# Keytoyze/Mug-Diffusion

Measured on NVIDIA H100. Metric: denoising-steps/sec, higher is better.
Workload: dtype f32

## Files before the change

### mug_diffusion_b200/csrc/gemm_tc.cu

```cuda
#include "gemm_tc.cuh"

namespace mugd {

template <int BN, int EPI>
__global__ void __launch_bounds__(TC_THREADS, 1)
gemm_tc_kernel(const __grid_constant__ CUtensorMap tmA, const __grid_constant__ CUtensorMap tmA1,
               const __grid_constant__ CUtensorMap tmA2, const __grid_constant__ CUtensorMap tmB, const __grid_constant__ CUtensorMap tmWhi,
               const __grid_constant__ CUtensorMap tmWlo, const __grid_constant__ TcParams p) {
    extern __shared__ uint8_t smem_raw[];
    const uint32_t base = (smem_u32(smem_raw) + 1023u) & ~1023u;
    const TcBars<BN> B(base);
    TC_STAMP(p, 0, blockIdx.x == 0 && blockIdx.y == 0 && blockIdx.z == 0);
    if (threadIdx.x < 32) {
        B.init_parallel((int)threadIdx.x);
    } else if (threadIdx.x < 38) {
        const CUtensorMap* m = threadIdx.x == 32 ? &tmA : threadIdx.x == 33 ? &tmA1 : threadIdx.x == 34 ? &tmA2
                             : threadIdx.x == 35 ? &tmB : threadIdx.x == 36 ? &tmWhi : &tmWlo;
        asm volatile("prefetch.tensormap [%0];" ::"l"(reinterpret_cast<uint64_t>(m)) : "memory");
    }
    __syncthreads();
    TC_STAMP(p, 1, blockIdx.x == 0 && blockIdx.y == 0 && blockIdx.z == 0);
    gemm_tc_tile<BN, EPI>(&tmA, &tmA1, &tmA2, &tmB, &tmWhi, &tmWlo, p, blockIdx.x, blockIdx.y, blockIdx.z, base);
}

template <int BN, int EPI>
__global__ void __launch_bounds__(TC_THREADS)
gemm_tc_reduce_kernel(const __grid_constant__ TcParams p) {
    tc_reduce<BN, EPI>(p, blockIdx.x);
}

#ifdef MUGD_TC_TIMELINE
static long long* g_tc_dbg = nullptr;
#endif
static float g_tc_kstep128 = 0.55f;
static float g_tc_split = 3.0f;
static int g_tc_force_bn = 0;

static bool tc_shape_ok(const mugd_gemm& g) {
    if (!(g.conv_mode == MUGD_CONV_NONE || g.conv_mode == MUGD_CONV_SAME || g.conv_mode == MUGD_CONV_DOWN ||
          g.conv_mode == MUGD_CONV_TAPS)) return false;
    if (g.conv_mode == MUGD_CONV_DOWN && g.Lout < 2) return false;
    if (g.K2 % TC_BK != 0 || (g.K2 > 0 && g.conv_mode == MUGD_CONV_DOWN)) return false;
    return g.K % TC_BK == 0 && g.N >= 16 && g.N % 4 == 0;
}

bool gemm_tc_supported(const mugd_gemm& g) {
    if (!tc_shape_ok(g)) return false;
    if (!g.W_hi || !g.W_lo) return false;
    if (g.lda % 4 != 0 || !aligned16(g.A) || !aligned16(g.W_hi) || !aligned16(g.W_lo)) return false;
    if (g.K2 > 0 && (!g.A2 || g.lda2 % 4 != 0 || !aligned16(g.A2))) return false;
    return true;
}

static int tc_validate_fusions(const mugd_gemm& g) {
    if (g.row_moments)
        MUGD_REQUIRE(g.act == MUGD_ACT_NONE && g.gate == MUGD_GATE_NONE && !g.ln_stats && (reinterpret_cast<uintptr_t>(g.row_moments) & 15u) == 0,
                     "gemm: row_moments needs act == gate == NONE, no folded LayerNorm and a 16-byte aligned buffer");
    if (g.ln_stats) {
        MUGD_REQUIRE(g.ln_colsum && aligned16(g.ln_colsum) && (reinterpret_cast<uintptr_t>(g.ln_stats) & 15u) == 0 && g.taps == 1 && g.K2 == 0 &&
                         g.act == MUGD_ACT_NONE && (g.gate == MUGD_GATE_NONE || g.gate == MUGD_GATE_GEGLU) && !g.rowvec,
                     "gemm: folded LayerNorm needs a single-source Linear with act NONE and gate NONE/GEGLU");
    }
    return MUGD_OK;
}

TcGeometry tc_geometry(const mugd_gemm& g, int sm_count, int forced_split) {
    TcGeometry t = {};
    TcParams::Hot& h = t.hot;
    t.BN = (g.N >= 128) ? 128 : 64;
    if (g.conv_mode == MUGD_CONV_NONE) { h.Lrows = g.M; h.Bs = 1; }
    else { h.Lrows = g.Lout; h.Bs = g.M / g.Lout; }
    if (h.Lrows >= TC_BM) {
        h.box_l = TC_BM; h.box_b = 1;
        h.tiles_per_sample = (h.Lrows + TC_BM - 1) / TC_BM;
        t.gy = h.tiles_per_sample * h.Bs;
    } else {
        h.box_l = h.Lrows;
        h.box_b = TC_BM / h.Lrows;
        if (h.box_b > h.Bs) h.box_b = h.Bs;
        h.tiles_per_sample = 1;
        t.gy = (h.Bs + h.box_b - 1) / h.box_b;
    }
    h.kblocks = g.K / TC_BK;
    h.it_main = g.taps * h.kblocks;
    h.total_it = h.it_main + g.K2 / TC_BK;
    int splits = 1;
    float best = 1e30f;
    static const int cands[2] = {64, 128};
    for (int cand = 0; cand < 2; ++cand) {
        const int bn = cands[cand];
        if (bn > 64 && g.N < bn) continue;
        if (bn == 64 && g.N >= 128 && g_tc_force_bn != 64) continue;
        if (g_tc_force_bn && bn != g_tc_force_bn && !(g_tc_force_bn > g.N && bn == 64)) continue;
        const int gx = (g.N + bn - 1) / bn;
        const int tiles = gx * t.gy;
        const float kstep = bn == 128 ? g_tc_kstep128 : 0.4f;
        const int sp_max = forced_split > 0 ? forced_split : (tiles < sm_count ? 16 : 1);
        for (int sp = forced_split > 0 ? forced_split : 1; sp <= sp_max && sp <= h.total_it; ++sp) {
            const int per = (h.total_it + sp - 1) / sp;
            if (forced_split <= 0 && sp > 1 && per < 2) break;
            if (forced_split <= 0 && sp > 1 && tiles * sp > 2 * sm_count) break;
            const int waves = (tiles * sp + sm_count - 1) / sm_count;
            const float est = waves * (1.0f + kstep * per) + (sp > 1 ? g_tc_split : 0.0f);
            if (est < best - 0.25f) { best = est; splits = sp; t.BN = bn; }
        }
    }
    h.gx = (g.N + t.BN - 1) / t.BN;
    if (splits > h.total_it) splits = h.total_it;
    if (splits < 1) splits = 1;
    h.splits = splits;
    h.it_base = h.total_it / splits;
    h.it_rem = h.total_it % splits;
    h.conv_mode = g.conv_mode;
    h.tap_shift = g.tap_shift;
    h.tap_dilation = g.tap_dilation;
    t.ws_floats = splits > 1 ? (int64_t)h.gx * t.gy * splits * TC_BM * t.BN : 0;
    return t;
}

int tc_plan(const DeviceInfo& dev, const mugd_gemm& g, const mugd_gemm* next, TcPlanned* out) {
    MUGD_REQUIRE(gemm_tc_supported(g), "gemm_tc: unsupported shape/operands");
    int rc = tc_validate_fusions(g);
    if (rc != MUGD_OK) return rc;
    const TcGeometry t = tc_geometry(g, dev.sm_count, g.split_k);
    const TcParams::Hot& h = t.hot;
    if (h.splits > 1) {
        MUGD_REQUIRE(g.workspace, "gemm_tc: split-K needs a workspace");
        MUGD_REQUIRE(g.workspace_bytes >= t.ws_floats * 4, "gemm_tc: workspace too small (%lld < %lld)", (long long)g.workspace_bytes,
                     (long long)t.ws_floats * 4);
    }
    const cuuint32_t a_box[3] = {(cuuint32_t)TC_BK, (cuuint32_t)h.box_l, (cuuint32_t)h.box_b};
    for (int tap = 0; tap < 3; ++tap) {
        if (tap > 0 && g.conv_mode != MUGD_CONV_DOWN) { out->maps[tap] = out->maps[0]; continue; }
        const bool down = g.conv_mode == MUGD_CONV_DOWN;
        const cuuint64_t rows = down ? (cuuint64_t)(h.Lrows - (tap == 2 ? 1 : 0)) : (cuuint64_t)h.Lrows;
        const cuuint64_t sample_rows = down ? (cuuint64_t)g.Lin : (cuuint64_t)h.Lrows;
        const cuuint64_t dims[3] = {(cuuint64_t)g.K, rows, (cuuint64_t)h.Bs};
        const cuuint64_t strides[2] = {(cuuint64_t)g.lda * 4 * (down ? 2 : 1), sample_rows * (cuuint64_t)g.lda * 4};
        rc = encode_f32_tma(&out->maps[tap], g.A + (down ? (int64_t)tap * g.lda : 0), 3, dims, strides, a_box, CU_TENSOR_MAP_L2_PROMOTION_L2_128B,
                            "gemm_tc A");
        if (rc != MUGD_OK) return rc;
    }
    if (g.K2 > 0) {
        const cuuint64_t dims[3] = {(cuuint64_t)g.K2, (cuuint64_t)h.Lrows, (cuuint64_t)h.Bs};
        const cuuint64_t strides[2] = {(cuuint64_t)g.lda2 * 4, (cuuint64_t)h.Lrows * (cuuint64_t)g.lda2 * 4};
        rc = encode_f32_tma(&out->maps[3], g.A2, 3, dims, strides, a_box, CU_TENSOR_MAP_L2_PROMOTION_L2_128B, "gemm_tc A2");
        if (rc != MUGD_OK) return rc;
    } else {
        out->maps[3] = out->maps[0];
    }
    const cuuint64_t ktot = (cuuint64_t)g.taps * g.K + g.K2;
    const cuuint64_t w_dims[2] = {ktot, (cuuint64_t)g.N};
    const cuuint64_t w_strides[1] = {ktot * 4};
    const cuuint32_t w_box[2] = {(cuuint32_t)TC_BK, (cuuint32_t)t.BN};
    for (int w = 0; w < 2; ++w) {
        rc = encode_f32_tma(&out->maps[4 + w], w == 0 ? g.W_hi : g.W_lo, 2, w_dims, w_strides, w_box, CU_TENSOR_MAP_L2_PROMOTION_L2_256B,
                            "gemm_tc W");
        if (rc != MUGD_OK) return rc;
    }
    TcParams& p = out->p;
    memset(&p, 0, sizeof(p));
    p.hot = h;
    p.hot.single_pass = dev.tc_single_pass ? 1 : 0;
    p.g = g;
    p.ws = (float*)g.workspace;
    p.gy = t.gy;
    p.ln_invK = 1.0 / (double)g.K;
    if (next) {
        p.pf_hi = next->W_hi;
        p.pf_lo = p.hot.single_pass ? nullptr : next->W_lo;
        p.pf_bytes = (int64_t)next->N * ((int64_t)next->taps * next->K + next->K2) * 4;
    }
#ifdef MUGD_TC_TIMELINE
    p.dbg = g_tc_dbg;
#endif
    out->BN = t.BN;
    return MUGD_OK;
}

template <int BN, int EPI>
static int tc_launch(const TcPlanned& pl, cudaStream_t st) {
    const TcParams& p = pl.p;
    const TcParams::Hot& h = p.hot;
    if (h.splits > 1) {
        MUGD_CHECK_CUDA(launch_k(gemm_tc_kernel<BN, TC_E_NONE>, dim3(h.gx, p.gy, h.splits), dim3(TC_THREADS), TcSmem<BN>::TOTAL, st, pl.maps[0],
                                 pl.maps[1], pl.maps[2], pl.maps[3], pl.maps[4], pl.maps[5], p));
        MUGD_CHECK_CUDA(launch_k(gemm_tc_reduce_kernel<BN, EPI>, dim3((unsigned)(h.gx * p.gy * (TC_BM / TC_RED_ROWS<BN>))), dim3(TC_THREADS), 0,
                                 st, p));
        return MUGD_OK;
    }
    MUGD_CHECK_CUDA(launch_k(gemm_tc_kernel<BN, EPI>, dim3(h.gx, p.gy, 1), dim3(TC_THREADS), TcSmem<BN>::TOTAL, st, pl.maps[0], pl.maps[1],
                             pl.maps[2], pl.maps[3], pl.maps[4], pl.maps[5], p));
    return MUGD_OK;
}

template <int BN, int... EPI>
static cudaError_t allow_smem_bn(int bytes, std::integer_sequence<int, EPI...>) {
    return allow_dynamic_smem(bytes, gemm_tc_kernel<BN, EPI>...);
}
cudaError_t gemm_tc_allow_smem(int bytes) {
    const cudaError_t e = allow_smem_bn<64>(bytes, std::make_integer_sequence<int, TC_E_COUNT>{});
    return e != cudaSuccess ? e : allow_smem_bn<128>(bytes, std::make_integer_sequence<int, TC_E_COUNT>{});
}

template <int BN>
static int tc_launch_bn(const TcPlanned& pl, cudaStream_t st) {
    switch (tc_epi_of(pl.p.g)) {
        case TC_E_GEGLU: return tc_launch<BN, TC_E_GEGLU>(pl, st);
        case TC_E_GLU: return tc_launch<BN, TC_E_GLU>(pl, st);
        case TC_E_SILU: return tc_launch<BN, TC_E_SILU>(pl, st);
        case TC_E_GELU: return tc_launch<BN, TC_E_GELU>(pl, st);
        case TC_E_SINK: return tc_launch<BN, TC_E_SINK>(pl, st);
        case TC_E_LN: return tc_launch<BN, TC_E_LN>(pl, st);
        case TC_E_LN_GEGLU: return tc_launch<BN, TC_E_LN_GEGLU>(pl, st);
        default: return tc_launch<BN, TC_E_NONE>(pl, st);
    }
}

int launch_gemm_tc(const DeviceInfo& dev, const mugd_gemm& g, const mugd_gemm* next, cudaStream_t st, int* launches) {
    TcPlanned pl;
    int rc = tc_plan(dev, g, next, &pl);
    if (rc != MUGD_OK) return rc;
    if (pl.BN == 128) rc = tc_launch_bn<128>(pl, st);
    else rc = tc_launch_bn<64>(pl, st);
    if (rc != MUGD_OK) return rc;
    if (launches) *launches += pl.p.hot.splits > 1 ? 2 : 1;
    return MUGD_OK;
}

}

extern "C" int mugd_debug_set_tc_cost(float kstep128_us, float kstep256_us, float split_us, float two_cta_fixed_us) {
    (void)kstep256_us;
    (void)two_cta_fixed_us;
    if (kstep128_us > 0.f) mugd::g_tc_kstep128 = kstep128_us;
    if (split_us > 0.f) mugd::g_tc_split = split_us;
    return MUGD_OK;
}

extern "C" int mugd_debug_set_tc_tile_n(int bn) {
    mugd::g_tc_force_bn = (bn == 64 || bn == 128) ? bn : 0;
    return MUGD_OK;
}

extern "C" int mugd_debug_set_tc_timing(long long* device_buf) {
#ifdef MUGD_TC_TIMELINE
    mugd::g_tc_dbg = device_buf;
    return MUGD_OK;
#else
    (void)device_buf;
    mugd::set_error("mugd_debug_set_tc_timing: this build has no timeline hooks (rebuild with -DMUGD_TC_TIMELINE, tools/build_variant.py)");
    return MUGD_ERR_INVALID;
#endif
}

extern "C" int mugd_gemm_tc_variant(const mugd_gemm* g, int32_t sm_count, int32_t* tile_n, int32_t* ctas_per_sm, int32_t* grid_ctas) {
    using namespace mugd;
    MUGD_REQUIRE(g, "gemm_tc_variant: null");
    if (!tc_shape_ok(*g)) {
        if (tile_n) *tile_n = 0;
        if (ctas_per_sm) *ctas_per_sm = 0;
        if (grid_ctas) *grid_ctas = 0;
        return MUGD_OK;
    }
    const int sms = sm_count > 0 ? sm_count : 132;
    const TcGeometry t = tc_geometry(*g, sms, g->split_k);
    if (tile_n) *tile_n = t.BN;
    if (ctas_per_sm) *ctas_per_sm = 1;
    if (grid_ctas) *grid_ctas = t.hot.gx * t.gy * t.hot.splits;
    return MUGD_OK;
}

extern "C" int mugd_gemm_tc_query(mugd_handle*, const mugd_gemm* g, int32_t sm_count, int32_t* supported, int32_t* splits,
                                  int64_t* workspace_bytes, int32_t* n_tiles) {
    using namespace mugd;
    MUGD_REQUIRE(g, "gemm_tc_query: null");
    const bool ok = tc_shape_ok(*g);
    if (supported) *supported = ok ? 1 : 0;
    if (!ok) {
        if (splits) *splits = 0;
        if (workspace_bytes) *workspace_bytes = 0;
        if (n_tiles) *n_tiles = 0;
        return MUGD_OK;
    }
    const TcGeometry t = tc_geometry(*g, sm_count > 0 ? sm_count : 132, g->split_k);
    if (splits) *splits = t.hot.splits;
    if (workspace_bytes) *workspace_bytes = t.ws_floats * 4;
    if (n_tiles) *n_tiles = t.hot.gx * t.gy;
    return MUGD_OK;
}
```

### mug_diffusion_b200/csrc/gemm_tc.cuh

```cuda
#pragma once
#include <cuda.h>
#include <stddef.h>

#include <type_traits>

#include "common.cuh"
#include "wgmma.cuh"

namespace mugd {

constexpr int TC_BM = 128;
constexpr int TC_BK = 32;
constexpr int TC_THREADS = 256;
constexpr uint32_t TC_A_BYTES = TC_BM * TC_BK * 4;

struct TcParams {
    struct Hot {
        int32_t Lrows, Bs;
        int32_t box_l, box_b;
        int32_t tiles_per_sample;
        int32_t it_base, it_rem;
        int32_t it_main;
        int32_t kblocks;
        int32_t total_it;
        int32_t splits;
        int32_t single_pass;
        int32_t conv_mode, tap_shift, tap_dilation;
        int32_t gx;
    } hot;
    mugd_gemm g;
    float* ws;
    int32_t gy;
    double ln_invK;
    const float* pf_hi;
    const float* pf_lo;
    int64_t pf_bytes;
#ifdef MUGD_TC_TIMELINE
    long long* dbg;
#endif
};
static_assert(sizeof(TcParams::Hot) == 64 && offsetof(TcParams, hot) == 0, "the hot fields are the first 64 bytes of the parameters");

#ifdef __CUDACC__
__device__ __forceinline__ long long gtimer() {
    long long t;
    asm volatile("mov.u64 %0, %%globaltimer;" : "=l"(t) :: "memory");
    return t;
}
#ifdef MUGD_TC_TIMELINE
#define TC_STAMP(p, k, cta0) do { if ((p).dbg && (cta0) && threadIdx.x == 0) (p).dbg[k] = gtimer(); } while (0)
#else
#define TC_STAMP(p, k, cta0) do { } while (0)
#endif
template <int BN>
struct TcSmem {
    static_assert(BN == 64 || BN == 128, "tile widths of the wgmma kernel");
    static constexpr uint32_t B_BYTES = BN * TC_BK * 4;
    static constexpr uint32_t STAGE_BYTES = TC_A_BYTES + 2 * B_BYTES;
    static constexpr int STAGES = BN == 128 ? 4 : 6;
    static constexpr uint32_t TILE_BYTES = STAGES * STAGE_BYTES;
    static constexpr uint32_t BAR_BYTES = 256;
    static constexpr uint32_t TOTAL = TILE_BYTES + 1024  + BAR_BYTES;
    static_assert(TOTAL <= 227u * 1024u, "shared memory budget");
    static_assert(128u * (BN + 4) * 4u + 1024u <= TILE_BYTES, "the staged accumulator tile + row statistics must fit the pipeline buffers");
};

template <int SEG>
__device__ __forceinline__ void tc_row_sink(double* buf, int m, float4 v) {
    float s = (v.x + v.y) + (v.z + v.w);
    float ss = (v.x * v.x + v.y * v.y) + (v.z * v.z + v.w * v.w);
#pragma unroll
    for (int o = SEG / 2; o > 0; o >>= 1) {
        s += __shfl_xor_sync(0xffffffffu, s, o);
        ss += __shfl_xor_sync(0xffffffffu, ss, o);
    }
    if ((threadIdx.x & (SEG - 1)) == 0 && m >= 0) {
        atomicAdd(buf + (int64_t)m * 2, (double)s);
        atomicAdd(buf + (int64_t)m * 2 + 1, (double)ss);
    }
}
__device__ __forceinline__ float2 tc_ln_from_moments(double s, double ss, double invK, float eps) {
    const double mean = s * invK;
    double var = ss * invK - mean * mean;
    const float v = fmaxf((float)var, 0.f) + eps;
    float r = rsqrtf(v);
    r = r * (1.5f - 0.5f * v * r * r);
    return make_float2((float)mean, r);
}

constexpr int TC_EPI_PLAIN = 0, TC_EPI_SINK = 1 , TC_EPI_LN = 2 ;

template <int ACT, int GATE, bool LNF>
__device__ __forceinline__ float4 tc_finish4(const mugd_gemm& g, float* dst, float4 acc, float4 bia, float4 rvv, float4 res, float4 cs, float2 ln,
                                             int m, int no) {
    float x[4];
    if constexpr (LNF) {
        x[0] = (acc.x - ln.x * cs.x) * ln.y + bia.x + rvv.x; x[1] = (acc.y - ln.x * cs.y) * ln.y + bia.y + rvv.y;
        x[2] = (acc.z - ln.x * cs.z) * ln.y + bia.z + rvv.z; x[3] = (acc.w - ln.x * cs.w) * ln.y + bia.w + rvv.w;
    } else {
        x[0] = acc.x + bia.x + rvv.x; x[1] = acc.y + bia.y + rvv.y; x[2] = acc.z + bia.z + rvv.z; x[3] = acc.w + bia.w + rvv.w;
    }
    if constexpr (ACT == MUGD_ACT_SILU) {
#pragma unroll
        for (int j = 0; j < 4; ++j) x[j] = silu_f(x[j]);
    } else if constexpr (ACT == MUGD_ACT_GELU) {
#pragma unroll
        for (int j = 0; j < 4; ++j) x[j] = gelu_f(x[j]);
    }
    if constexpr (GATE == MUGD_GATE_NONE) {
        const float4 o = make_float4(x[0] + res.x, x[1] + res.y, x[2] + res.z, x[3] + res.w);
        st_f4(dst, o);
        return o;
    } else {
        float o0, o1;
        if constexpr (GATE == MUGD_GATE_GEGLU) { o0 = x[0] * gelu_f(x[1]); o1 = x[2] * gelu_f(x[3]); }
        else { o0 = x[0] * sigmoid_f(x[1]); o1 = x[2] * sigmoid_f(x[3]); }
        if (g.residual) {
            const float2 rr = *reinterpret_cast<const float2*>(g.residual + (int64_t)m * g.ldr + no);
            o0 += rr.x; o1 += rr.y;
        }
        *reinterpret_cast<float2*>(dst) = make_float2(o0, o1);
        return make_float4(o0, o1, 0.f, 0.f);
    }
}

template <int BN, int ACT, int GATE, int MODE>
__device__ __forceinline__ void tc_store_tile(const mugd_gemm& g, uint32_t stage, int m_base, int n0, int rows_valid, const float* rowvec,
                                              uint32_t rowstat, float4 bia, float4 cs) {
    constexpr int SP = BN + 4;
    constexpr int C4 = BN / 4;
    constexpr int NU = TC_BM * C4 / TC_THREADS;
    constexpr int U = NU < 16 ? NU : 16;
    constexpr int SEG = C4 < 32 ? C4 : 32;
    static_assert(TC_THREADS % C4 == 0, "a thread keeps its column quad for the whole tile");
    const int c4 = (int)threadIdx.x % C4;
    const int nn = n0 + c4 * 4;
    const bool col_ok = nn < g.N;
    const bool has_res = GATE == MUGD_GATE_NONE && g.residual != nullptr;
    constexpr int RPP = TC_THREADS / C4;
    const int row0 = (int)threadIdx.x / C4;
    const int n_rows = min(rows_valid, g.M - m_base);
    const int no = (GATE == MUGD_GATE_NONE) ? nn : (nn >> 1);
    float* cp = g.C + (int64_t)(m_base + row0) * g.ldc + no;
    const float* rp = has_res ? g.residual + (int64_t)(m_base + row0) * g.ldr + nn : nullptr;
    const int64_t c_step = (int64_t)RPP * g.ldc, r_step = (int64_t)RPP * g.ldr;
    int smp = 0, smp_end = 0;
    if (rowvec) { smp = (m_base + row0) / g.Lout; smp_end = (smp + 1) * g.Lout; }
    auto pass = [&](auto full_tag) {
        constexpr bool FULL = decltype(full_tag)::value;
#pragma unroll 1
        for (int i0 = 0; i0 < NU; i0 += U) {
            float4 res[U], rvv[U];
#pragma unroll
            for (int u = 0; u < U; ++u) {
                const int row = row0 + (i0 + u) * RPP;
                res[u] = rvv[u] = make_float4(0.f, 0.f, 0.f, 0.f);
                if (FULL || (row < n_rows && col_ok)) {
                    if (has_res) res[u] = ld_f4(rp + (int64_t)(i0 + u) * r_step);
                    if (rowvec) {
                        const int m = m_base + row;
                        while (m >= smp_end) { ++smp; smp_end += g.Lout; }
                        rvv[u] = ld_f4(rowvec + (int64_t)smp * g.rowvec_b_stride + nn);
                    }
                }
            }
#pragma unroll
            for (int u = 0; u < U; ++u) {
                const int row = row0 + (i0 + u) * RPP;
                const int m = m_base + row;
                const bool ok = FULL || (row < n_rows && col_ok);
                const float4 acc = lds_f4(stage + (uint32_t)(row * SP + c4 * 4) * 4u);
                float2 ln = make_float2(0.f, 1.f);
                if constexpr (MODE == TC_EPI_LN) ln = lds_f2(rowstat + (uint32_t)row * 8u);
                float4 o = make_float4(0.f, 0.f, 0.f, 0.f);
                if (ok) o = tc_finish4<ACT, GATE, MODE == TC_EPI_LN>(g, cp + (int64_t)(i0 + u) * c_step, acc, bia, rvv[u], res[u], cs, ln, m, no);
                if constexpr (MODE == TC_EPI_SINK) tc_row_sink<SEG>(g.row_moments, ok ? m : -1, o);
            }
        }
    };
    if (n_rows >= TC_BM && n0 + BN <= g.N) pass(std::true_type{});
    else pass(std::false_type{});
}

enum TcEpi { TC_E_NONE = 0, TC_E_GEGLU, TC_E_GLU, TC_E_SILU, TC_E_GELU, TC_E_SINK, TC_E_LN, TC_E_LN_GEGLU, TC_E_COUNT };
template <int EPI> struct TcEpiTraits;
template <> struct TcEpiTraits<TC_E_NONE>     { static constexpr int ACT = MUGD_ACT_NONE, GATE = MUGD_GATE_NONE,  MODE = TC_EPI_PLAIN; };
template <> struct TcEpiTraits<TC_E_GEGLU>    { static constexpr int ACT = MUGD_ACT_NONE, GATE = MUGD_GATE_GEGLU, MODE = TC_EPI_PLAIN; };
template <> struct TcEpiTraits<TC_E_GLU>      { static constexpr int ACT = MUGD_ACT_NONE, GATE = MUGD_GATE_GLU,   MODE = TC_EPI_PLAIN; };
template <> struct TcEpiTraits<TC_E_SILU>     { static constexpr int ACT = MUGD_ACT_SILU, GATE = MUGD_GATE_NONE,  MODE = TC_EPI_PLAIN; };
template <> struct TcEpiTraits<TC_E_GELU>     { static constexpr int ACT = MUGD_ACT_GELU, GATE = MUGD_GATE_NONE,  MODE = TC_EPI_PLAIN; };
template <> struct TcEpiTraits<TC_E_SINK>     { static constexpr int ACT = MUGD_ACT_NONE, GATE = MUGD_GATE_NONE,  MODE = TC_EPI_SINK; };
template <> struct TcEpiTraits<TC_E_LN>       { static constexpr int ACT = MUGD_ACT_NONE, GATE = MUGD_GATE_NONE,  MODE = TC_EPI_LN; };
template <> struct TcEpiTraits<TC_E_LN_GEGLU> { static constexpr int ACT = MUGD_ACT_NONE, GATE = MUGD_GATE_GEGLU, MODE = TC_EPI_LN; };

inline int tc_epi_of(const mugd_gemm& g) {
    if (g.ln_stats) return g.gate == MUGD_GATE_GEGLU ? TC_E_LN_GEGLU : TC_E_LN;
    if (g.row_moments) return TC_E_SINK;
    if (g.gate == MUGD_GATE_GEGLU) return TC_E_GEGLU;
    if (g.gate == MUGD_GATE_GLU) return TC_E_GLU;
    if (g.act == MUGD_ACT_SILU) return TC_E_SILU;
    if (g.act == MUGD_ACT_GELU) return TC_E_GELU;
    return TC_E_NONE;
}

__device__ __forceinline__ void tc_tile_rows(const TcParams& p, int by, int& b_base, int& l_base, int& rows_valid) {
    const TcParams::Hot& h = p.hot;
    if (h.Lrows >= TC_BM) {
        b_base = by / h.tiles_per_sample;
        l_base = (by % h.tiles_per_sample) * TC_BM;
        rows_valid = min(TC_BM, h.Lrows - l_base);
    } else {
        b_base = by * h.box_b;
        l_base = 0;
        rows_valid = min(h.box_b, h.Bs - b_base) * h.Lrows;
    }
}

template <int BN>
struct TcBars {
    using S = TcSmem<BN>;
    static constexpr int COUNT = 2 * S::STAGES;
    static_assert(8 * COUNT <= (int)S::BAR_BYTES, "barrier block");
    uint32_t bars;
    __device__ __forceinline__ explicit TcBars(uint32_t base) : bars(base + S::TILE_BYTES) {}
    __device__ __forceinline__ uint32_t full(int s) const { return bars + 8u * s; }
    __device__ __forceinline__ uint32_t empty(int s) const { return bars + 8u * (S::STAGES + s); }
    __device__ __forceinline__ void init_parallel(int t) const {
        if (t >= COUNT) return;
        mbar_init(bars + 8u * t, t < S::STAGES ? 1u : (uint32_t)(TC_THREADS / 32));
        mbar_init_fence();
    }
};

struct TcAFrag {
    uint32_t hi[4][4], lo[4][4];
};
__device__ __forceinline__ void tc_load_split(uint32_t a_tile, int r0, int t, TcAFrag& f) {
#pragma unroll
    for (int kk = 0; kk < 4; ++kk) {
#pragma unroll
        for (int e = 0; e < 4; ++e) {
            const int r = r0 + (e & 1) * 8;
            const int chunk = 2 * kk + (e >> 1);
            const float x = lds_f1(a_tile + (uint32_t)r * 128u + (uint32_t)((chunk ^ (r & 7)) << 4) + (uint32_t)t * 4u);
            const float h = to_tf32(x);
            f.hi[kk][e] = __float_as_uint(h);
            f.lo[kk][e] = __float_as_uint(to_tf32(x - h));
        }
    }
}

template <int BN, int EPI>
__device__ __forceinline__ void gemm_tc_tile(const CUtensorMap* tmA, const CUtensorMap* tmA1, const CUtensorMap* tmA2, const CUtensorMap* tmB,
                                             const CUtensorMap* tmWhi, const CUtensorMap* tmWlo, const TcParams& p, int bx, int by, int bz,
                                             uint32_t base) {
    using S = TcSmem<BN>;
    constexpr int STAGES = S::STAGES;
    constexpr int NACC = BN / 2;
    const TcBars<BN> B(base);
    auto a_raw = [&](int s) { return base + s * S::STAGE_BYTES; };
    auto b_hi = [&](int s) { return base + s * S::STAGE_BYTES + TC_A_BYTES; };
    auto b_lo = [&](int s) { return b_hi(s) + S::B_BYTES; };

    const mugd_gemm& g = p.g;
    const TcParams::Hot& h = p.hot;
    const int warp = threadIdx.x >> 5, lane = threadIdx.x & 31;
    const int n0 = bx * BN;
    int b_base, l_base, rows_valid;
    tc_tile_rows(p, by, b_base, l_base, rows_valid);
    const int m_base = b_base * h.Lrows + l_base;
    const int it_begin = bz * h.it_base + min(bz, h.it_rem);
    const int nit = h.it_base + (bz < h.it_rem ? 1 : 0);
    const uint32_t a_tx = (uint32_t)(h.box_l * h.box_b) * TC_BK * 4;
    const uint32_t w_tx = (h.single_pass ? 1u : 2u) * S::B_BYTES;

    auto issue_w = [&](int i) {
        const int s = i % STAGES, it = it_begin + i;
        mbar_expect_tx(B.full(s), a_tx + w_tx);
        tma_load_2d(b_hi(s), tmWhi, B.full(s), it * TC_BK, n0);
        if (!h.single_pass) tma_load_2d(b_lo(s), tmWlo, B.full(s), it * TC_BK, n0);
    };
    auto issue_a = [&](int i) {
        const int s = i % STAGES, it = it_begin + i;
        if (it < h.it_main) {
            const int t = it / h.kblocks;
            const int kb = it - t * h.kblocks;
            const CUtensorMap* ma = tmA;
            int lshift = 0;
            if (h.conv_mode == MUGD_CONV_SAME) lshift = t - 1;
            else if (h.conv_mode == MUGD_CONV_TAPS) lshift = (t + h.tap_shift) * (h.tap_dilation > 1 ? h.tap_dilation : 1);
            else if (h.conv_mode == MUGD_CONV_DOWN) ma = (t == 0) ? tmA : (t == 1 ? tmA1 : tmA2);
            tma_load_3d(a_raw(s), ma, B.full(s), kb * TC_BK, l_base + lshift, b_base);
        } else {
            tma_load_3d(a_raw(s), tmB, B.full(s), (it - h.it_main) * TC_BK, l_base, b_base);
        }
    };
    if (warp == 0) {
        if (elect_one()) {
            const int pro = nit < STAGES ? nit : STAGES;
            for (int i = 0; i < pro; ++i) issue_w(i);
            pdl_wait();
            for (int i = 0; i < pro; ++i) issue_a(i);
            if (p.pf_bytes > 0) {
                const int64_t ncta = (int64_t)h.gx * p.gy * h.splits;
                const int64_t per = (p.pf_bytes / ncta + 15) & ~(int64_t)15;
                const int64_t off = (((int64_t)bz * p.gy + by) * h.gx + bx) * per;
                const int64_t n = min(per, p.pf_bytes - off);
                if (n > 0) {
                    prefetch_l2(reinterpret_cast<const char*>(p.pf_hi) + off, (uint32_t)n);
                    if (p.pf_lo) prefetch_l2(reinterpret_cast<const char*>(p.pf_lo) + off, (uint32_t)n);
                }
            }
        }
        __syncwarp();
    }

    int epi_step = 0;
    float4 epi_bias = make_float4(0.f, 0.f, 0.f, 0.f), epi_cs = epi_bias;
    double ln_s = 0.0, ln_ss = 0.0;
    {
        pdl_wait();
        if (h.splits == 1) {
            const int nn = n0 + ((int)threadIdx.x % (BN / 4)) * 4;
            if (g.step) epi_step = *g.step;
            if (g.bias && nn < g.N) epi_bias = ld_f4(g.bias + nn);
            if constexpr (TcEpiTraits<EPI>::MODE == TC_EPI_LN) {
                if (nn < g.N) epi_cs = ld_f4(g.ln_colsum + nn);
            }
        }
        if constexpr (TcEpiTraits<EPI>::MODE == TC_EPI_LN) {
            const int rr = (int)threadIdx.x;
            if (rr < TC_BM && rr < rows_valid && m_base + rr < g.M) {
                const double2 mo = *reinterpret_cast<const double2*>(g.ln_stats + (int64_t)m_base * 2 + rr * 2);
                ln_s = mo.x; ln_ss = mo.y;
            }
        }
    }

    const int wg = warp >> 2, g8 = lane >> 2, t4 = lane & 3;
    const int r0 = wg * 64 + (warp & 3) * 16 + g8;
    float acc[NACC];
#pragma unroll
    for (int j = 0; j < NACC; ++j) acc[j] = 0.f;
    TcAFrag f0, f1;
    if (nit > 0) {
        mbar_wait(B.full(0), 0u);
        tc_load_split(a_raw(0), r0, t4, f0);
    }
    auto main_loop = [&](auto single_tag) {
        constexpr bool SINGLE = decltype(single_tag)::value;
        auto kstep = [&](int i, const TcAFrag& cur, TcAFrag& nxt) {
            const int s = i % STAGES;
            const uint64_t dbh = wgmma_desc(b_hi(s)), dbl = wgmma_desc(b_lo(s));
            wgmma_fence();
#pragma unroll
            for (int kk = 0; kk < TC_BK / 8; ++kk) {
                const uint64_t ko = (uint64_t)(kk * 2);
                if constexpr (SINGLE) {
                    Wgmma<BN>::mma(acc, cur.hi[kk], dbh + ko);
                } else {
                    Wgmma<BN>::mma(acc, cur.lo[kk], dbh + ko);
                    Wgmma<BN>::mma(acc, cur.hi[kk], dbl + ko);
                    Wgmma<BN>::mma(acc, cur.hi[kk], dbh + ko);
                }
            }
            wgmma_commit();
            wgmma_wait<1>();
            if (i > 0) {
                const int j = i - 1, sj = j % STAGES;
                __syncwarp();
                if (lane == 0) mbar_arrive(B.empty(sj));
                if (warp == 0 && j + STAGES < nit) {
                    mbar_wait(B.empty(sj), (uint32_t)(j / STAGES) & 1u);
                    if (elect_one()) { issue_w(j + STAGES); issue_a(j + STAGES); }
                    __syncwarp();
                }
            }
            if (i + 1 < nit) {
                mbar_wait(B.full((i + 1) % STAGES), (uint32_t)((i + 1) / STAGES) & 1u);
                tc_load_split(a_raw((i + 1) % STAGES), r0, t4, nxt);
            }
        };
        for (int i = 0; i < nit; i += 2) {
            kstep(i, f0, f1);
            if (i + 1 < nit) kstep(i + 1, f1, f0);
        }
    };
    if (h.single_pass) main_loop(std::true_type{});
    else main_loop(std::false_type{});
    wgmma_wait<0>();
    TC_STAMP(p, 2, bx == 0 && by == 0 && bz == 0);
    float2 lnrow = make_float2(0.f, 1.f);
    if constexpr (TcEpiTraits<EPI>::MODE == TC_EPI_LN) lnrow = tc_ln_from_moments(ln_s, ln_ss, p.ln_invK, g.ln_eps);
    __syncthreads();
    constexpr int SP = BN + 4;
#pragma unroll
    for (int j = 0; j < BN / 8; ++j) {
        const int c = j * 8 + 2 * t4;
        sts_f2(base + (uint32_t)(r0 * SP + c) * 4u, acc[4 * j], acc[4 * j + 1]);
        sts_f2(base + (uint32_t)((r0 + 8) * SP + c) * 4u, acc[4 * j + 2], acc[4 * j + 3]);
    }
    if constexpr (TcEpiTraits<EPI>::MODE == TC_EPI_LN) {
        if (threadIdx.x < TC_BM) sts_f2(base + S::TILE_BYTES - 1024u + (uint32_t)threadIdx.x * 8u, lnrow.x, lnrow.y);
    }
    __syncthreads();
    TC_STAMP(p, 3, bx == 0 && by == 0 && bz == 0);
    {
        const float* rowvec = g.rowvec ? g.rowvec + (int64_t)epi_step * g.rowvec_step_stride : nullptr;
        if (h.splits > 1) {
            const int tile_lin = by * h.gx + bx;
            float* wsp = p.ws + ((int64_t)tile_lin * h.splits + bz) * (TC_BM * BN);
            constexpr int C4 = BN / 4;
            constexpr int U = 8;
#pragma unroll 1
            for (int i0 = 0; i0 < TC_BM * C4; i0 += TC_THREADS * U) {
                float4 a4[U];
#pragma unroll
                for (int u = 0; u < U; ++u) {
                    const int idx = i0 + u * TC_THREADS + (int)threadIdx.x;
                    const int row = idx / C4, c4 = idx - row * C4;
                    a4[u] = lds_f4(base + (uint32_t)(row * SP + c4 * 4) * 4u);
                }
#pragma unroll
                for (int u = 0; u < U; ++u) st_f4(wsp + (i0 + u * TC_THREADS + (int)threadIdx.x) * 4, a4[u]);
            }
        } else {
            using E = TcEpiTraits<EPI>;
            tc_store_tile<BN, E::ACT, E::GATE, E::MODE>(g, base, m_base, n0, rows_valid, rowvec, base + S::TILE_BYTES - 1024u, epi_bias, epi_cs);
        }
    }
    TC_STAMP(p, 4, bx == 0 && by == 0 && bz == 0);
}

template <int BN> constexpr int TC_RED_ROWS = TC_THREADS / (BN / 4);

template <int BN, int EPI>
__device__ __forceinline__ void tc_reduce(const TcParams& p, int blk) {
    constexpr int ACT = TcEpiTraits<EPI>::ACT, GATE = TcEpiTraits<EPI>::GATE, MODE = TcEpiTraits<EPI>::MODE;
    constexpr int C4 = BN / 4;
    constexpr int BPT = TC_BM / TC_RED_ROWS<BN>;
    constexpr int SEG = C4 < 32 ? C4 : 32;
    constexpr int ZU = 8;
    const mugd_gemm& g = p.g;
    const TcParams::Hot& h = p.hot;
    const int tile_lin = blk / BPT;
    const int bx = tile_lin % h.gx, by = tile_lin / h.gx;
    int b_base, l_base, rows_valid;
    tc_tile_rows(p, by, b_base, l_base, rows_valid);
    const int m_base = b_base * h.Lrows + l_base;
    const int c4 = (int)threadIdx.x % C4;
    const int r = (blk % BPT) * TC_RED_ROWS<BN> + (int)threadIdx.x / C4;
    const int n = bx * BN + c4 * 4;
    const int m = m_base + r;
    const bool ok = r < rows_valid && m < g.M && n < g.N;
    float4 bia = make_float4(0.f, 0.f, 0.f, 0.f), rvv = bia, res = bia, cs = bia;
    if (ok && g.bias) bia = ld_f4(g.bias + n);
    if constexpr (MODE == TC_EPI_LN) {
        if (ok) cs = ld_f4(g.ln_colsum + n);
    }
    pdl_wait();
    int step = 0;
    if (g.step) step = *g.step;
    if (GATE == MUGD_GATE_NONE && g.residual && ok) res = ld_f4(g.residual + (int64_t)m * g.ldr + n);
    double2 mo = make_double2(0.0, 1.0);
    if constexpr (MODE == TC_EPI_LN) {
        if (ok) mo = *reinterpret_cast<const double2*>(g.ln_stats + (int64_t)m * 2);
    }
    const float* src = p.ws + ((long long)tile_lin * h.splits) * (TC_BM * BN) + (long long)r * BN + c4 * 4;
    float4 acc = make_float4(0.f, 0.f, 0.f, 0.f);
    for (int z0 = 0; z0 < h.splits; z0 += ZU) {
        float4 t4[ZU];
#pragma unroll
        for (int u = 0; u < ZU; ++u) {
            t4[u] = make_float4(0.f, 0.f, 0.f, 0.f);
            if (ok && z0 + u < h.splits) t4[u] = __ldcg(reinterpret_cast<const float4*>(src + (long long)(z0 + u) * (TC_BM * BN)));
        }
        if (z0 == 0 && g.rowvec && ok)
            rvv = ld_f4(g.rowvec + (int64_t)step * g.rowvec_step_stride + (int64_t)(m / g.Lout) * g.rowvec_b_stride + n);
#pragma unroll
        for (int u = 0; u < ZU; ++u) { acc.x += t4[u].x; acc.y += t4[u].y; acc.z += t4[u].z; acc.w += t4[u].w; }
    }
    float4 o = make_float4(0.f, 0.f, 0.f, 0.f);
    if (ok) {
        float2 ln = make_float2(0.f, 1.f);
        if constexpr (MODE == TC_EPI_LN) ln = tc_ln_from_moments(mo.x, mo.y, p.ln_invK, g.ln_eps);
        const int no = (GATE == MUGD_GATE_NONE) ? n : (n >> 1);
        o = tc_finish4<ACT, GATE, MODE == TC_EPI_LN>(g, g.C + (int64_t)m * g.ldc + no, acc, bia, rvv, res, cs, ln, m, no);
    }
    if constexpr (MODE == TC_EPI_SINK) tc_row_sink<SEG>(g.row_moments, ok ? m : -1, o);
}

#endif

struct TcGeometry {
    TcParams::Hot hot;
    int BN, gy;
    int64_t ws_floats;
};
struct alignas(64) TcPlanned {
    CUtensorMap maps[6];
    TcParams p;
    int BN;
};
TcGeometry tc_geometry(const mugd_gemm& g, int sm_count, int forced_split);
int tc_plan(const DeviceInfo& dev, const mugd_gemm& g, const mugd_gemm* next, TcPlanned* out);

}
```

Measured before the change: 246.8.

## Recalibrate split-K cost model with L2 traffic and store partials directly from registers

The split/BN selection heuristic now uses microsecond-scale fill and per-k-step costs, a much cheaper split penalty, and an L2 traffic term estimated from operand re-reads and split-K partial writes. Split-K CTAs now write their accumulator fragments straight from registers to the workspace, skipping the shared-memory staging round trip and its barriers. This likely makes split-K chosen more often for small-tile GEMMs, trading extra workspace traffic and reduce launches for better SM fill. The direct float2 stores are less coalesced than the previous float4 staging path.

New measurement: 246.6 (median of 6 runs). No clear change (-0.1%).

```diff
diff --git a/mug_diffusion_b200/csrc/gemm_tc.cu b/mug_diffusion_b200/csrc/gemm_tc.cu
--- a/mug_diffusion_b200/csrc/gemm_tc.cu
+++ b/mug_diffusion_b200/csrc/gemm_tc.cu
@@ -32,8 +32,11 @@
 #ifdef MUGD_TC_TIMELINE
 static long long* g_tc_dbg = nullptr;
 #endif
-static float g_tc_kstep128 = 0.55f;
-static float g_tc_split = 3.0f;
+static float g_tc_kstep128 = 0.70f;
+static float g_tc_split = 0.78f;
+static constexpr float TC_FILL_US = 4.90f;
+static constexpr float TC_KSTEP64_US = 0.52f;
+static constexpr double TC_US_PER_BYTE = 3.0e-8;
 static int g_tc_force_bn = 0;
 
 static bool tc_shape_ok(const mugd_gemm& g) {
@@ -62,6 +65,12 @@
                      "gemm: folded LayerNorm needs a single-source Linear with act NONE and gate NONE/GEGLU");
     }
     return MUGD_OK;
+}
+
+double tc_l2_bytes(int64_t M, int64_t N, int64_t Kt, int bn, int gy, int splits) {
+    const int64_t gx = (N + bn - 1) / bn;
+    const double part = splits > 1 ? (double)gx * gy * splits * TC_BM * bn * 8 : 0.0;
+    return (double)M * Kt * 4 * gx + (double)N * Kt * 8 * gy + part;
 }
 
 TcGeometry tc_geometry(const mugd_gemm& g, int sm_count, int forced_split) {
@@ -94,14 +103,15 @@
         if (g_tc_force_bn && bn != g_tc_force_bn && !(g_tc_force_bn > g.N && bn == 64)) continue;
         const int gx = (g.N + bn - 1) / bn;
         const int tiles = gx * t.gy;
-        const float kstep = bn == 128 ? g_tc_kstep128 : 0.4f;
+        const float kstep = bn == 128 ? g_tc_kstep128 : TC_KSTEP64_US;
         const int sp_max = forced_split > 0 ? forced_split : (tiles < sm_count ? 16 : 1);
         for (int sp = forced_split > 0 ? forced_split : 1; sp <= sp_max && sp <= h.total_it; ++sp) {
             const int per = (h.total_it + sp - 1) / sp;
             if (forced_split <= 0 && sp > 1 && per < 2) break;
             if (forced_split <= 0 && sp > 1 && tiles * sp > 2 * sm_count) break;
             const int waves = (tiles * sp + sm_count - 1) / sm_count;
-            const float est = waves * (1.0f + kstep * per) + (sp > 1 ? g_tc_split : 0.0f);
+            const float est = waves * (TC_FILL_US + kstep * per) + (sp > 1 ? g_tc_split : 0.0f) +
+                              (float)(TC_US_PER_BYTE * tc_l2_bytes(g.M, g.N, g.taps * g.K + g.K2, bn, t.gy, sp));
             if (est < best - 0.25f) { best = est; splits = sp; t.BN = bn; }
         }
     }
diff --git a/mug_diffusion_b200/csrc/gemm_tc.cuh b/mug_diffusion_b200/csrc/gemm_tc.cuh
--- a/mug_diffusion_b200/csrc/gemm_tc.cuh
+++ b/mug_diffusion_b200/csrc/gemm_tc.cuh
@@ -392,6 +392,18 @@
     TC_STAMP(p, 2, bx == 0 && by == 0 && bz == 0);
     float2 lnrow = make_float2(0.f, 1.f);
     if constexpr (TcEpiTraits<EPI>::MODE == TC_EPI_LN) lnrow = tc_ln_from_moments(ln_s, ln_ss, p.ln_invK, g.ln_eps);
+    if (h.splits > 1) {
+        float* wsp = p.ws + ((int64_t)(by * h.gx + bx) * h.splits + bz) * (TC_BM * BN);
+#pragma unroll
+        for (int j = 0; j < BN / 8; ++j) {
+            const int c = j * 8 + 2 * t4;
+            *reinterpret_cast<float2*>(wsp + r0 * BN + c) = make_float2(acc[4 * j], acc[4 * j + 1]);
+            *reinterpret_cast<float2*>(wsp + (r0 + 8) * BN + c) = make_float2(acc[4 * j + 2], acc[4 * j + 3]);
+        }
+        TC_STAMP(p, 3, bx == 0 && by == 0 && bz == 0);
+        TC_STAMP(p, 4, bx == 0 && by == 0 && bz == 0);
+        return;
+    }
     __syncthreads();
     constexpr int SP = BN + 4;
 #pragma unroll
@@ -407,27 +419,8 @@
     TC_STAMP(p, 3, bx == 0 && by == 0 && bz == 0);
     {
         const float* rowvec = g.rowvec ? g.rowvec + (int64_t)epi_step * g.rowvec_step_stride : nullptr;
-        if (h.splits > 1) {
-            const int tile_lin = by * h.gx + bx;
-            float* wsp = p.ws + ((int64_t)tile_lin * h.splits + bz) * (TC_BM * BN);
-            constexpr int C4 = BN / 4;
-            constexpr int U = 8;
-#pragma unroll 1
-            for (int i0 = 0; i0 < TC_BM * C4; i0 += TC_THREADS * U) {
-                float4 a4[U];
-#pragma unroll
-                for (int u = 0; u < U; ++u) {
-                    const int idx = i0 + u * TC_THREADS + (int)threadIdx.x;
-                    const int row = idx / C4, c4 = idx - row * C4;
-                    a4[u] = lds_f4(base + (uint32_t)(row * SP + c4 * 4) * 4u);
-                }
-#pragma unroll
-                for (int u = 0; u < U; ++u) st_f4(wsp + (i0 + u * TC_THREADS + (int)threadIdx.x) * 4, a4[u]);
-            }
-        } else {
-            using E = TcEpiTraits<EPI>;
-            tc_store_tile<BN, E::ACT, E::GATE, E::MODE>(g, base, m_base, n0, rows_valid, rowvec, base + S::TILE_BYTES - 1024u, epi_bias, epi_cs);
-        }
+        using E = TcEpiTraits<EPI>;
+        tc_store_tile<BN, E::ACT, E::GATE, E::MODE>(g, base, m_base, n0, rows_valid, rowvec, base + S::TILE_BYTES - 1024u, epi_bias, epi_cs);
     }
     TC_STAMP(p, 4, bx == 0 && by == 0 && bz == 0);
 }
@@ -502,6 +495,7 @@
     TcParams p;
     int BN;
 };
+double tc_l2_bytes(int64_t M, int64_t N, int64_t Kt, int bn, int gy, int splits);
 TcGeometry tc_geometry(const mugd_gemm& g, int sm_count, int forced_split);
 int tc_plan(const DeviceInfo& dev, const mugd_gemm& g, const mugd_gemm* next, TcPlanned* out);
 
```
